# PeterouZh/CIPS-3Dplusplus

Hardware: AMD Instinct MI355X
Metric: rendered views/sec at FFHQ 1024^2 (generator forward: 64x64-ray NeRF + StyleGAN2 decoder) (higher is better)
Workload: dtype f32 (split-fp16 MFMA products x3, f32 accumulate and storage); 1 GPU; ffhq_r1024_nerf64x64x24_D2_B1_fp32; img_size=64, n_samples=24, N_layers_renderer=2, resolution=1024, parallelism=views x1, views_in_flight=2

## Files before the change

### cips_3dplusplus_amd/csrc/fused_stage.hip

```cpp

#include <type_traits>

#include "up2_fir.h"

namespace {

struct FusedArgs {
  const float* y_lo; const float* fir; const float* noise1; int64_t nbs1; const float* nw1; const float* bias1;
  const float* wm2; const float* noise2; int64_t nbs2; const float* nw2; const float* bias2; float* out2;
  const float* wm_rgb; const float* bias_rgb; const float* skip; int skip_up; float* rgb;
  int B, H, W;
  int bf16;
  const float* wm_next; float* y_next;
  const float* x_amax; const float* lconst1; const float* lconst2; float* next_amax;
  float next_gain;
  int flat;
};

#ifndef CIPS3D_FUSED_AB
#define CIPS3D_FUSED_AB 0
#endif
#ifdef CIPS3D_FUSED_STAMPS
__device__ unsigned long long g_fused_stamps[4][8];
#define FSTAMP(i) do { const unsigned long long t_ = __builtin_amdgcn_s_memtime(); fst_[i] += t_ - ftp_; ftp_ = t_; } while (0)
#define FSTAMP_FLUSH() do { if (tid == 0 && (blockIdx.x & 31) == 0) {    constexpr int sl_ = C == 32 ? 0 : C == 64 ? 1 : C == 128 ? 2 : 3; \
    for (int i_ = 0; i_ < 7; ++i_) atomicAdd(&g_fused_stamps[sl_][i_], fst_[i_]); atomicAdd(&g_fused_stamps[sl_][7], 1ull); } } while (0)
#else
#define FSTAMP(i)
#define FSTAMP_FLUSH()
#endif

template <int C, int WM, int WGM, int WGN, int RW, int BK, int MINW, int PREC, bool NEXT = false, bool XPREF = false,
          bool LATE_OPS = false, bool FLAT = false>
__global__ void __launch_bounds__(64 * WGM * WGN, MINW) fused_up_conv_kernel(FusedArgs a) {
  constexpr bool BF16 = PREC == 1 || PREC == 2;
  constexpr bool YB = PREC == 2;
  constexpr bool SPLIT = PREC == 3;
  typedef typename std::conditional<YB, bf16_t, float>::type ylo_t;
  constexpr int NT = 64 * WGM * WGN;
  constexpr int CW = 64 / RW, TH = RW * WGN, TW = CW, BN = TH * TW;
  constexpr int NSTAGE = C / BK, NBUF = NSTAGE > 1 ? 2 : 1, KQ = BK / 16;
  constexpr int LPR = CW / 4;
  static_assert((WGM * WGN == 8 || WGM * WGN == 4) && 16 * WM * WGM == C && TH % 2 == 0 && C % BK == 0, "tile shape");
  constexpr int NBLK = (TH / 2) * (TW / 4);
  constexpr int BPT = BK * NBLK / NT;
  static_assert((BK * NBLK) % NT == 0 && BPT >= 1, "block split");
  __shared__ __attribute__((aligned(16))) float sB[NBUF * BK * BN];
  __shared__ __attribute__((aligned(16))) float s_nz1[BN + 8];
  __shared__ __attribute__((aligned(16))) float s_red_own[NEXT ? WGM * 3 * BN : 4];
  float* s_red = NEXT ? s_red_own : sB;
  __shared__ __attribute__((aligned(16))) float s_wrgb[3 * C];

  const int tid = threadIdx.x;
#ifdef CIPS3D_FUSED_STAMPS
  unsigned long long fst_[7] = {0, 0, 0, 0, 0, 0, 0}, ftp_ = __builtin_amdgcn_s_memtime();
#endif
  const int wave = __builtin_amdgcn_readfirstlane(tid >> 6);
  const int lane = tid & 63;
  const int wm_i = wave / WGN, wn_i = wave % WGN;
  const int q = lane >> 4, jn = lane & 15;
  const int lrow = jn / LPR, lx4 = jn % LPR;
  const int nloc = (wn_i * RW + lrow) * TW + lx4 * 4;
  const int b = blockIdx.z;
  const int H = a.H, W = a.W, OH = FLAT ? H : 2 * H, OW = FLAT ? W : 2 * W;
  const int tiles_x = OW / TW;
  int bid = blockIdx.x;
  if ((gridDim.x & 7) == 0) bid = (bid & 7) * (gridDim.x >> 3) + (bid >> 3);
  const int ox0 = (bid % tiles_x) * TW, oy0 = (bid / tiles_x) * TH;
  const int HWlo = H * W, HWo = OH * OW;
  const int oy = oy0 + wn_i * RW + lrow, ox = ox0 + lx4 * 4;

  float kact1 = 1.41421356237309515f, k2in = kSplitInv, kact2 = 1.41421356237309515f, kback2 = 1.f, kyn = kSplitInv;

  float nw1_u = 0.f;
  float c10_u = 0.f, c11_u = 0.f, c20_u = 0.f, c21a_u = 0.f, c21b_u = 0.f;
  if constexpr (SPLIT) {
    if (a.x_amax && !(CIPS3D_FUSED_AB & 1)) {
      const float* l1 = a.lconst1 + b * 4;
      c10_u = l1[0]; c11_u = l1[1];
      if (NEXT) {
        const float* l2 = a.lconst2 + b * 4;
        c20_u = l2[0]; c21a_u = l2[1]; c21b_u = l2[2];
      }
    }
  }
  const float* ab = a.wm2 + (int64_t)b * C * C;
  f32x4 afr_next[KQ][WM];
#pragma unroll
  for (int kq = 0; kq < KQ; ++kq)
#pragma unroll
    for (int i = 0; i < WM; ++i)
      afr_next[kq][i] = *reinterpret_cast<const f32x4*>(ab + (((wm_i * WM + i) * (C / 16) + kq) * 256 + lane * 4));
  constexpr bool LATE = LATE_OPS;
  f32x4 nz2 = {0.f, 0.f, 0.f, 0.f};
  float nw2_u = 0.f;
  f32x4 bias4[WM];
  auto load_epilogue_ops = [&]() {
    if (a.noise2 && a.nw2 && !(CIPS3D_FUSED_AB & 128)) {
      nz2 = *reinterpret_cast<const f32x4*>(a.noise2 + (int64_t)b * a.nbs2 + (oy * OW + ox));
      nw2_u = a.nw2[0];
    }
#pragma unroll
    for (int i = 0; i < WM; ++i) bias4[i] = *reinterpret_cast<const f32x4*>(a.bias2 + (wm_i * WM + i) * 16 + 4 * q);
  };
  if (!LATE) load_epilogue_ops();

  float kf[16];
#pragma unroll
  for (int i = 0; i < 16; ++i) kf[i] = FLAT ? 0.f : a.fir[15 - i];
  const bool rgb_lane = a.wm_rgb && wm_i == 0 && q < 3;
  float skp[3][4];
  f32x4 skv = {0.f, 0.f, 0.f, 0.f};
  float rgb_bias = 0.f;
  auto load_skip_ops = [&]() {
    if (rgb_lane) {
      rgb_bias = a.bias_rgb[q];
      if (a.skip && !(CIPS3D_FUSED_AB & 128)) {
        if (!FLAT && (a.skip_up & 1)) up2_load(a.skip + (int64_t)b * 3 * HWlo + q * HWlo, H, W, oy >> 1, ox >> 2, skp);
        else skv = *reinterpret_cast<const f32x4*>(a.skip + (int64_t)b * 3 * HWo + (q * HWo + oy * OW + ox));
      }
    }
  };
  if (!LATE) load_skip_ops();

  const bool interior = FLAT || (oy0 / 2 >= 1 && oy0 / 2 + TH / 2 < H && ox0 / 2 >= 1 && ox0 / 2 + TW / 2 < W);
  constexpr bool DEEP = NSTAGE >= 3 && C >= 256;
  float pv[BPT][3][4], pw[BPT][3][4];
  auto patch_load_into = [&](int st, float (&pset)[BPT][3][4]) {
#pragma unroll
    for (int u = 0; u < BPT; ++u) {
      const int g = tid + NT * u;
      const int ch = g / NBLK, rem = g % NBLK;
      const int by = rem / (TW / 4), qx = rem % (TW / 4);
      const ylo_t* src = reinterpret_cast<const ylo_t*>(a.y_lo) + (int64_t)b * C * HWlo + (st * BK + ch) * HWlo;
      if constexpr (CIPS3D_FUSED_AB & 64) {
#pragma unroll
        for (int r = 0; r < 3; ++r)
#pragma unroll
          for (int c = 0; c < 4; ++c) pset[u][r][c] = __int_as_float(0x3c000000 + ((tid + st + r * 4 + c) << 8));
      } else
      if constexpr (FLAT) flat_load(src, W, oy0 + 2 * by, ox0 + 4 * qx, pset[u]);
      else if (interior) up2_load_interior(src, W, oy0 / 2 + by, ox0 / 4 + qx, pset[u]);
      else up2_load(src, H, W, oy0 / 2 + by, ox0 / 4 + qx, pset[u]);
    }
  };
  auto patch_load = [&](int st) { patch_load_into(st, pv); };
  auto patch_store_from = [&](int st, float* dst, float (&pset)[BPT][3][4]) {
#pragma unroll
    for (int u = 0; u < BPT; ++u) {
      const int g = tid + NT * u;
      const int ch = g / NBLK, rem = g % NBLK;
      const int by = rem / (TW / 4), qx = rem % (TW / 4);
      float o[2][4];
      if constexpr (FLAT) {
#pragma unroll
        for (int c = 0; c < 4; ++c) { o[0][c] = pset[u][0][c]; o[1][c] = pset[u][1][c]; }
      } else if constexpr (CIPS3D_FUSED_AB & 8) {
#pragma unroll
        for (int c = 0; c < 4; ++c) { o[0][c] = pset[u][0][c] + pset[u][1][c]; o[1][c] = pset[u][1][c] + pset[u][2][c]; }
      } else {
        up2_fir(pset[u], kf, o);
      }
      const float bs = a.bias1[st * BK + ch];
#pragma unroll
      for (int py = 0; py < 2; ++py) {
        const f32x4 nz = *reinterpret_cast<const f32x4*>(s_nz1 + (2 * by + py) * TW + qx * 4);
        f32x4 v;
#pragma unroll
        for (int c = 0; c < 4; ++c) {
          const float on = fmaf(nw1_u, nz[c], o[py][c]);
          v[c] = (CIPS3D_FUSED_AB & 32) ? on : lrelu02(on + bs);
        }
        if constexpr (SPLIT && !(CIPS3D_FUSED_AB & 32)) {
#pragma unroll
          for (int c = 0; c < 4; ++c) v[c] = pack_split(v[c], kact1);
        } else {
#pragma unroll
          for (int c = 0; c < 4; ++c) v[c] *= kact1;
        }
        *reinterpret_cast<f32x4*>(dst + ch * BN + (2 * by + py) * TW + qx * 4) = v;
      }
    }
  };
  auto patch_store = [&](int st, float* dst) { patch_store_from(st, dst, pv); };
  patch_load(0);
  if (DEEP) patch_load_into(1, pw);
  const bool have_nz = a.noise1 && a.nw1 && !(CIPS3D_FUSED_AB & 128);
  if (have_nz) nw1_u = a.nw1[0];
  if (wave == 0) {
    static_assert(BN / 4 <= 64 && (3 * C) % 4 == 0, "one LDS-DMA instruction per tile");
    if (lane < BN / 4) {
      if (have_nz) {
        const int r = lane / (TW / 4), x4 = lane % (TW / 4);
        __builtin_amdgcn_global_load_lds((const __attribute__((address_space(1))) void*)(a.noise1 + (int64_t)b * a.nbs1 + ((oy0 + r) * OW + ox0 + x4 * 4)),
                                         (__attribute__((address_space(3))) void*)s_nz1, 16, 0, 0);
      } else {
        *reinterpret_cast<f32x4*>(s_nz1 + lane * 4) = f32x4{0.f, 0.f, 0.f, 0.f};
      }
    }
  }
  if (a.wm_rgb) {
#pragma unroll
    for (int p0 = 0; p0 < 3 * C / 4; p0 += 64 * WGM * WGN) {
      const int pbase = p0 + wave * 64;
      if (pbase < 3 * C / 4 && pbase + lane < 3 * C / 4)
        __builtin_amdgcn_global_load_lds((const __attribute__((address_space(1))) void*)(a.wm_rgb + (int64_t)b * 3 * C + (pbase + lane) * 4),
                                         (__attribute__((address_space(3))) void*)(s_wrgb + pbase * 4), 16, 0, 0);
    }
  }


  if constexpr (SPLIT) {
    if (a.x_amax && wave == 0 && !(CIPS3D_FUSED_AB & 1)) {
      const float t = lane < CIPS3D_AMAX_SLOTS ? a.x_amax[b * CIPS3D_AMAX_FLOATS + lane * CIPS3D_AMAX_STRIDE] : 0.f;
      float c10 = c10_u, c11 = c11_u, c20 = 0.f, c21 = 0.f;
      if (NEXT) { c20 = c20_u; c21 = fmaxf(c21a_u, 1.41421356237309515f * c21b_u); }
      if (FLAT) c11 = 1.41421356237309515f;
      const float m_in = cips3d_wave_max_uniform(t);
      const float u1 = fmaf(c11, m_in, c10);
      const int e1 = cips3d_split_exp(u1);
      f32x4 sc = {1.41421356237309515f * cips3d_pow2(-e1), kSplitInv * cips3d_pow2(e1), 1.41421356237309515f, 1.f};
      if (NEXT) {
        const float u2 = fmaf(c21, u1, c20);
        const int e2 = cips3d_split_exp(u2);
        sc[2] = 1.41421356237309515f * cips3d_pow2(-e2);
        sc[3] = cips3d_pow2(e2);
        if (a.next_amax && a.next_gain > 0.f && blockIdx.x == 0 && lane == 0) a.next_amax[b * CIPS3D_AMAX_FLOATS] = a.next_gain * u2 * 1.000001f;
      }
      if (lane == 0) *reinterpret_cast<f32x4*>(s_nz1 + BN) = sc;
    }
  }
  __builtin_amdgcn_s_waitcnt(0x0F70);
  __syncthreads();

  f32x4 acc[WM][4];
#pragma unroll
  for (int i = 0; i < WM; ++i)
#pragma unroll
    for (int c = 0; c < 4; ++c) acc[i][c] = f32x4{0.f, 0.f, 0.f, 0.f};

  FSTAMP(0);
  if constexpr (SPLIT) {
    if (a.x_amax && !(CIPS3D_FUSED_AB & 1)) {
      const f32x4 sc = *reinterpret_cast<const f32x4*>(s_nz1 + BN);
      kact1 = cips3d_uniform(sc[0]);
      k2in = cips3d_uniform(sc[1]);
      if (NEXT) {
        kact2 = cips3d_uniform(sc[2]);
        kback2 = cips3d_uniform(sc[3]);
        kyn = cips3d_uniform(kSplitInv * kback2);
      }
    }
  }

  patch_store(0, sB);
  __syncthreads();
  FSTAMP(1);
#pragma unroll (DEEP ? NSTAGE : 1)
  for (int st = 0; st < NSTAGE; ++st) {
    const float* cur = sB + (NBUF > 1 ? (st & 1) : 0) * BK * BN + nloc;
    f32x4 afr[KQ][WM];
#pragma unroll
    for (int kq = 0; kq < KQ; ++kq)
#pragma unroll
      for (int i = 0; i < WM; ++i) afr[kq][i] = afr_next[kq][i];
    if (st + 1 < NSTAGE) {
#pragma unroll
      for (int kq = 0; kq < KQ; ++kq)
#pragma unroll
        for (int i = 0; i < WM; ++i)
          afr_next[kq][i] = *reinterpret_cast<const f32x4*>(
              ab + (((wm_i * WM + i) * (C / 16) + (st + 1) * KQ + kq) * 256 + lane * 4));
      if (!DEEP) patch_load(st + 1);
    }
    if (DEEP && st + 2 < NSTAGE) {
      if (st & 1) patch_load_into(st + 2, pw);
      else patch_load_into(st + 2, pv);
    }
#pragma unroll
    for (int kq = 0; kq < KQ; ++kq) {
      if (BF16) {
        f32x4 b4[4];
#pragma unroll
        for (int j4 = 0; j4 < 4; ++j4) b4[j4] = *reinterpret_cast<const f32x4*>(cur + (kq * 16 + j4 * 4 + q) * BN);
        s16x4 ah[WM], bh[4];
#pragma unroll
        for (int i = 0; i < WM; ++i) ah[i] = pack_bf16(afr[kq][i][0], afr[kq][i][1], afr[kq][i][2], afr[kq][i][3]);
#pragma unroll
        for (int c = 0; c < 4; ++c) bh[c] = pack_bf16(b4[0][c], b4[1][c], b4[2][c], b4[3][c]);
#pragma unroll
        for (int i = 0; i < WM; ++i)
#pragma unroll
          for (int c = 0; c < 4; ++c)
            acc[i][c] = __builtin_amdgcn_mfma_f32_16x16x16bf16_1k(ah[i], bh[c], acc[i][c], 0, 0, 0);
      } else if constexpr (SPLIT) {
        f32x4 b4[4];
#pragma unroll
        for (int j4 = 0; j4 < 4; ++j4) b4[j4] = *reinterpret_cast<const f32x4*>(cur + (kq * 16 + j4 * 4 + q) * BN);
#pragma unroll
        for (int c = 0; c < 4; ++c) {
          h4 bh, bl;
          unpack_frag(b4[0][c], b4[1][c], b4[2][c], b4[3][c], bh, bl);
#pragma unroll
          for (int i = 0; i < WM; ++i) acc[i][c] = split_mfma16(afr[kq][i], bh, bl, acc[i][c]);
        }
      } else {
#pragma unroll
      for (int j4 = 0; j4 < 4; ++j4) {
        const f32x4 b4 = *reinterpret_cast<const f32x4*>(cur + (kq * 16 + j4 * 4 + q) * BN);
#pragma unroll
        for (int i = 0; i < WM; ++i)
#pragma unroll
          for (int c = 0; c < 4; ++c)
            acc[i][c] = fused_mfma(afr[kq][i][j4], b4[c], acc[i][c]);
      }
      }
    }
    if (NBUF > 1 && st + 1 < NSTAGE) {
      if (DEEP && ((st + 1) & 1)) patch_store_from(st + 1, sB + ((st + 1) & 1) * BK * BN, pw);
      else patch_store(st + 1, sB + ((st + 1) & 1) * BK * BN);
    }
    __syncthreads();
  }

  FSTAMP(2);
  if (LATE) { load_epilogue_ops(); load_skip_ops(); }
  float prgb[3][4];
  float mxn = 0.f;
#pragma unroll
  for (int ch = 0; ch < 3; ++ch)
#pragma unroll
    for (int c = 0; c < 4; ++c) prgb[ch][c] = 0.f;
#pragma unroll
  for (int i = 0; i < WM; ++i) {
    const int obase = (wm_i * WM + i) * 16 + 4 * q;
#pragma unroll
    for (int r = 0; r < 4; ++r) {
      f32x4 v = {acc[i][0][r], acc[i][1][r], acc[i][2][r], acc[i][3][r]};
      if constexpr (SPLIT) {
#pragma unroll
        for (int c = 0; c < 4; ++c) v[c] *= k2in;
      }
#pragma unroll
      for (int c = 0; c < 4; ++c) v[c] = (CIPS3D_FUSED_AB & 16) ? v[c] : lrelu02(fmaf(nw2_u, nz2[c], v[c]) + bias4[i][r]) * kact2;
      if (NEXT) {
#pragma unroll
        for (int c = 0; c < 4; ++c) acc[i][c][r] = v[c];
      }
      if (a.out2) {
        if constexpr (NEXT && SPLIT) {
          *reinterpret_cast<f32x4*>(a.out2 + (int64_t)b * C * HWo + ((obase + r) * HWo + oy * OW + ox)) =
              f32x4{v[0] * kback2, v[1] * kback2, v[2] * kback2, v[3] * kback2};
        } else {
          *reinterpret_cast<f32x4*>(a.out2 + (int64_t)b * C * HWo + ((obase + r) * HWo + oy * OW + ox)) = v;
        }
      }
      if (a.wm_rgb && !(CIPS3D_FUSED_AB & 4)) {
#pragma unroll
        for (int ch = 0; ch < 3; ++ch) {
          const float w = s_wrgb[ch * C + obase + r];
#pragma unroll
          for (int c = 0; c < 4; ++c) prgb[ch][c] = fmaf(w, v[c], prgb[ch][c]);
        }
      }
    }
  }
  FSTAMP(3);
  constexpr int OTN = NEXT ? C / 32 : 1;
  constexpr bool XCHG = NEXT && XPREF && OTN % WGM == 0 && WGM % 2 == 0;
  if (XCHG) {
    constexpr int GR = (WGM / 2) * WM;
    constexpr int TPW = XCHG ? OTN / WGM : 1;
    static_assert(!XCHG || WGN * GR * 4 * 256 <= NBUF * BK * BN, "half of the activations must fit the B stages");
    const float* an = a.wm_next + (int64_t)b * (C / 2) * C + lane * 4;
    float* sx = sB + wn_i * GR * 4 * 256 + lane * 4;
    f32x4 accx[TPW][4];
#pragma unroll
    for (int tp = 0; tp < TPW; ++tp)
#pragma unroll
      for (int c = 0; c < 4; ++c) accx[tp][c] = f32x4{0.f, 0.f, 0.f, 0.f};
#pragma unroll
    for (int rd = 0; rd < 2; ++rd) {
      f32x4 af[TPW][GR];
#pragma unroll
      for (int tp = 0; tp < TPW; ++tp)
#pragma unroll
        for (int gl = 0; gl < GR; ++gl)
          af[tp][gl] = *reinterpret_cast<const f32x4*>(an + ((wm_i * TPW + tp) * (C / 16) + rd * GR + gl) * 256);
      if (wm_i / (WGM / 2) == rd) {
#pragma unroll
        for (int i = 0; i < WM; ++i)
#pragma unroll
          for (int r = 0; r < 4; ++r)
            *reinterpret_cast<f32x4*>(sx + (((wm_i % (WGM / 2)) * WM + i) * 4 + r) * 256) =
                SPLIT ? f32x4{pack_split(acc[i][0][r]), pack_split(acc[i][1][r]), pack_split(acc[i][2][r]), pack_split(acc[i][3][r])}
                      : f32x4{acc[i][0][r], acc[i][1][r], acc[i][2][r], acc[i][3][r]};
      }
      __syncthreads();
#pragma unroll
      for (int gl = 0; gl < GR; ++gl) {
        f32x4 bv[4];
#pragma unroll
        for (int r = 0; r < 4; ++r) bv[r] = *reinterpret_cast<const f32x4*>(sx + (gl * 4 + r) * 256);
        if (BF16) {
          s16x4 bh[4];
#pragma unroll
          for (int c = 0; c < 4; ++c) bh[c] = pack_bf16(bv[0][c], bv[1][c], bv[2][c], bv[3][c]);
#pragma unroll
          for (int tp = 0; tp < TPW; ++tp) {
            const s16x4 ah = pack_bf16(af[tp][gl][0], af[tp][gl][1], af[tp][gl][2], af[tp][gl][3]);
#pragma unroll
            for (int c = 0; c < 4; ++c) accx[tp][c] = __builtin_amdgcn_mfma_f32_16x16x16bf16_1k(ah, bh[c], accx[tp][c], 0, 0, 0);
          }
        } else if constexpr (SPLIT) {
#pragma unroll
          for (int c = 0; c < 4; ++c) {
            h4 bh, bl;
            unpack_frag(bv[0][c], bv[1][c], bv[2][c], bv[3][c], bh, bl);
#pragma unroll
            for (int tp = 0; tp < TPW; ++tp) accx[tp][c] = split_mfma16(af[tp][gl], bh, bl, accx[tp][c]);
          }
        } else {
#pragma unroll
          for (int r = 0; r < 4; ++r)
#pragma unroll
            for (int tp = 0; tp < TPW; ++tp)
#pragma unroll
              for (int c = 0; c < 4; ++c)
                accx[tp][c] = fused_mfma(af[tp][gl][r], bv[r][c], accx[tp][c]);
        }
      }
      __syncthreads();
    }
#pragma unroll
    for (int tp = 0; tp < TPW; ++tp) {
      ylo_t* yn = reinterpret_cast<ylo_t*>(a.y_next) + (int64_t)b * (C / 2) * HWo + (((wm_i * TPW + tp) * 16 + 4 * q) * HWo + oy * OW + ox);
#pragma unroll
      for (int r = 0; r < 4; ++r) {
        const float ys = SPLIT ? kyn : 1.f;
        const f32x4 yv = {accx[tp][0][r] * ys, accx[tp][1][r] * ys, accx[tp][2][r] * ys, accx[tp][3][r] * ys};
        mxn = fmaxf(fmaxf(fmaxf(fabsf(yv[0]), fabsf(yv[1])), fmaxf(fabsf(yv[2]), fabsf(yv[3]))), mxn);
        if constexpr (YB) cips3d_store_wt8(yn + r * HWo, pack_bf16(yv[0], yv[1], yv[2], yv[3]));
        else cips3d_store_wt16(yn + r * HWo, yv);
      }
    }
    if (a.next_amax && !(a.next_gain > 0.f) && !(CIPS3D_FUSED_AB & 2)) {
      static_assert(!NEXT || 4 * WGM * WGN <= BN, "the reduction words fit the noise tile");
      const float m = cips3d_workgroup_max(mxn, s_nz1, wave, lane, WGM * WGN);
      if (tid == 0) cips3d_amax_raise_if(a.next_amax + b * CIPS3D_AMAX_FLOATS, m, blockIdx.x);
    }
  }
  f32x4 accn[OTN][4];
  if (NEXT && !XCHG) {
    static_assert(!NEXT || XCHG || (WGM - 1) * WGN * OTN * 4 * 64 * 4 <= NBUF * BK * BN * 4, "split-K partials must fit the B stages");
    const float* an = a.wm_next + (int64_t)b * (C / 2) * C;
    f32x4 afn[OTN][WM];
#pragma unroll
    for (int t = 0; t < OTN; ++t)
#pragma unroll
      for (int i = 0; i < WM; ++i)
        afn[t][i] = *reinterpret_cast<const f32x4*>(an + ((t * (C / 16) + wm_i * WM + i) * 256 + lane * 4));
#pragma unroll
    for (int t = 0; t < OTN; ++t)
#pragma unroll
      for (int c = 0; c < 4; ++c) accn[t][c] = f32x4{0.f, 0.f, 0.f, 0.f};
#pragma unroll
    for (int i = 0; i < WM; ++i) {
      if (BF16) {
        s16x4 bh[4], ah[OTN];
#pragma unroll
        for (int c = 0; c < 4; ++c) bh[c] = pack_bf16(acc[i][c][0], acc[i][c][1], acc[i][c][2], acc[i][c][3]);
#pragma unroll
        for (int t = 0; t < OTN; ++t) ah[t] = pack_bf16(afn[t][i][0], afn[t][i][1], afn[t][i][2], afn[t][i][3]);
#pragma unroll
        for (int t = 0; t < OTN; ++t)
#pragma unroll
          for (int c = 0; c < 4; ++c) accn[t][c] = __builtin_amdgcn_mfma_f32_16x16x16bf16_1k(ah[t], bh[c], accn[t][c], 0, 0, 0);
      } else if constexpr (SPLIT) {
#pragma unroll
        for (int c = 0; c < 4; ++c) {
          h4 bh, bl;
          split_frag(acc[i][c][0], acc[i][c][1], acc[i][c][2], acc[i][c][3], bh, bl);
#pragma unroll
          for (int t = 0; t < OTN; ++t) accn[t][c] = split_mfma16(afn[t][i], bh, bl, accn[t][c]);
        }
      } else {
#pragma unroll
        for (int r = 0; r < 4; ++r)
#pragma unroll
          for (int t = 0; t < OTN; ++t)
#pragma unroll
            for (int c = 0; c < 4; ++c)
              accn[t][c] = fused_mfma(afn[t][i][r], acc[i][c][r], accn[t][c]);
      }
    }
    if (wm_i > 0) {
      float* sp = sB + ((((wm_i - 1) * WGN + wn_i) * OTN * 4) * 256 + lane * 4);
#pragma unroll
      for (int t = 0; t < OTN; ++t)
#pragma unroll
        for (int c = 0; c < 4; ++c) *reinterpret_cast<f32x4*>(sp + (t * 4 + c) * 256) = accn[t][c];
    }
  }
  FSTAMP(4);
  if (!a.wm_rgb && !NEXT) { FSTAMP_FLUSH(); return; }
  if (a.wm_rgb) {
    if constexpr (MINW >= 8) {
#pragma unroll
      for (int ch = 0; ch < 3; ++ch)
#pragma unroll
        for (int c = 0; c < 4; ++c) {
          float v = prgb[ch][c];
          v += __shfl_xor(v, 16, 64);
          v += __shfl_xor(v, 32, 64);
          prgb[ch][c] = (NEXT && SPLIT) ? v * kback2 : v;
        }
      if (q == 0) {
#pragma unroll
        for (int ch = 0; ch < 3; ++ch)
          *reinterpret_cast<f32x4*>(s_red + (wm_i * 3 + ch) * BN + nloc) =
              f32x4{prgb[ch][0], prgb[ch][1], prgb[ch][2], prgb[ch][3]};
      }
    } else {
    f32x4 tot;
#pragma unroll
    for (int c = 0; c < 4; ++c) {
      const auto rg = __builtin_amdgcn_permlane16_swap(__float_as_uint(prgb[0][c]), __float_as_uint(prgb[1][c]), false, false);
      const auto bb = __builtin_amdgcn_permlane16_swap(__float_as_uint(prgb[2][c]), __float_as_uint(prgb[2][c]), false, false);
      const float p = __uint_as_float(rg[0]) + __uint_as_float(rg[1]);
      const float u = __uint_as_float(bb[0]) + __uint_as_float(bb[1]);
      const auto h = __builtin_amdgcn_permlane32_swap(__float_as_uint(p), __float_as_uint(u), false, false);
      const float v = __uint_as_float(h[0]) + __uint_as_float(h[1]);
      tot[c] = (NEXT && SPLIT) ? v * kback2 : v;
    }
    if (q < 3) *reinterpret_cast<f32x4*>(s_red + (wm_i * 3 + q) * BN + nloc) = tot;
    }
  }
  __syncthreads();
  if (NEXT && !XCHG && wm_i == 0) {
#pragma unroll
    for (int m = 1; m < WGM; ++m) {
      const float* sp = sB + ((((m - 1) * WGN + wn_i) * OTN * 4) * 256 + lane * 4);
#pragma unroll
      for (int t = 0; t < OTN; ++t)
#pragma unroll
        for (int c = 0; c < 4; ++c) {
          const f32x4 pv4 = *reinterpret_cast<const f32x4*>(sp + (t * 4 + c) * 256);
#pragma unroll
          for (int r = 0; r < 4; ++r) accn[t][c][r] += pv4[r];
        }
    }
    ylo_t* yn = reinterpret_cast<ylo_t*>(a.y_next) + (int64_t)b * (C / 2) * HWo + (oy * OW + ox);
#pragma unroll
    for (int t = 0; t < OTN; ++t)
#pragma unroll
      for (int r = 0; r < 4; ++r) {
        const float ys = SPLIT ? kyn : 1.f;
        const f32x4 yv = {accn[t][0][r] * ys, accn[t][1][r] * ys, accn[t][2][r] * ys, accn[t][3][r] * ys};
        mxn = fmaxf(fmaxf(fmaxf(fabsf(yv[0]), fabsf(yv[1])), fmaxf(fabsf(yv[2]), fabsf(yv[3]))), mxn);
        if constexpr (YB) cips3d_store_wt8(yn + (t * 16 + 4 * q + r) * HWo, pack_bf16(yv[0], yv[1], yv[2], yv[3]));
        else cips3d_store_wt16(yn + (t * 16 + 4 * q + r) * HWo, yv);
      }
  }
  if (NEXT && !XCHG && a.next_amax && !(a.next_gain > 0.f) && !(CIPS3D_FUSED_AB & 2)) {
    const float m = cips3d_workgroup_max(mxn, s_nz1, wave, lane, WGM * WGN);
    if (tid == 0) cips3d_amax_raise_if(a.next_amax + b * CIPS3D_AMAX_FLOATS, m, blockIdx.x);
  }
  FSTAMP(5);
  if (!a.wm_rgb) { FSTAMP_FLUSH(); return; }
  if (rgb_lane) {
    const int ch = q;
    f32x4 v = {0.f, 0.f, 0.f, 0.f};
#pragma unroll
    for (int m = 0; m < WGM; ++m) {
      const f32x4 t = *reinterpret_cast<const f32x4*>(s_red + (m * 3 + ch) * BN + nloc);
#pragma unroll
      for (int c = 0; c < 4; ++c) v[c] += t[c];
    }
#pragma unroll
    for (int c = 0; c < 4; ++c) v[c] += rgb_bias;
    if (a.skip) {
      if (!FLAT && (a.skip_up & 1)) {
        float so[2][4];
        up2_fir(skp, kf, so);
        const int py = oy & 1;
#pragma unroll
        for (int c = 0; c < 4; ++c) v[c] += py ? so[1][c] : so[0][c];
      } else {
#pragma unroll
        for (int c = 0; c < 4; ++c) v[c] += skv[c];
      }
    }
    if (a.skip_up & 2) {
      unsigned pk = 0;
#pragma unroll
      for (int c = 0; c < 4; ++c) {
        const float cl = fminf(fmaxf(v[c], -1.f), 1.f);
        pk |= (unsigned)__float2int_rn((cl + 1.f) * 127.5f) << (8 * c);
      }
      *reinterpret_cast<unsigned*>(reinterpret_cast<unsigned char*>(a.rgb) + (int64_t)b * 3 * HWo + (ch * HWo + oy * OW + ox)) = pk;
    } else {
      cips3d_store_wt16(a.rgb + (int64_t)b * 3 * HWo + (ch * HWo + oy * OW + ox), v);
    }
  }
  FSTAMP(6);
  FSTAMP_FLUSH();
}

template <int C, int WM, int WGM, int WGN, int RW, int BK, int MINW, bool NEXT, bool XPREF, bool LATE, bool FLAT>
int launch_fused_as(const FusedArgs& a, hipStream_t st) {
  constexpr int TH = RW * WGN, TW = 64 / RW;
  const int up = FLAT ? 1 : 2;
  dim3 grid((unsigned)((up * a.W / TW) * (up * a.H / TH)), 1, (unsigned)a.B);
  if (a.bf16 == 3) hipLaunchKernelGGL((fused_up_conv_kernel<C, WM, WGM, WGN, RW, BK, MINW, 3, NEXT, XPREF, LATE, FLAT>), grid, dim3(64 * WGM * WGN), 0, st, a);
  else if (a.bf16 == 2) hipLaunchKernelGGL((fused_up_conv_kernel<C, WM, WGM, WGN, RW, BK, MINW, 2, NEXT, XPREF, LATE, FLAT>), grid, dim3(64 * WGM * WGN), 0, st, a);
  else if (a.bf16) hipLaunchKernelGGL((fused_up_conv_kernel<C, WM, WGM, WGN, RW, BK, MINW, 1, NEXT, XPREF, LATE, FLAT>), grid, dim3(64 * WGM * WGN), 0, st, a);
  else hipLaunchKernelGGL((fused_up_conv_kernel<C, WM, WGM, WGN, RW, BK, MINW, 0, NEXT, XPREF, LATE, FLAT>), grid, dim3(64 * WGM * WGN), 0, st, a);
  return cips3d_launch_status();
}
template <int C, int WM, int WGM, int WGN, int RW, int BK, int MINW, bool NEXT = false, bool XPREF = false, bool LATE = false>
int launch_fused(const FusedArgs& a, hipStream_t st) {
  return a.flat ? launch_fused_as<C, WM, WGM, WGN, RW, BK, MINW, NEXT, XPREF, LATE, true>(a, st)
                : launch_fused_as<C, WM, WGM, WGN, RW, BK, MINW, NEXT, XPREF, LATE, false>(a, st);
}

}

#ifdef CIPS3D_FUSED_STAMPS
extern "C" int cips3d_debug_read_fused_stamps(unsigned long long* out32) {
  hipDeviceSynchronize();
  hipMemcpyFromSymbol(out32, HIP_SYMBOL(g_fused_stamps), 256);
  unsigned long long z[32] = {0};
  hipMemcpyToSymbol(HIP_SYMBOL(g_fused_stamps), z, 256);
  return 0;
}
#endif

extern "C" int cips3d_fused_up_conv_supported(int C, int H, int W) {
  return (C == 32 || C == 64 || C == 128 || C == 256) && W % 32 == 0 && H % 2 == 0 && H >= 2 &&
         (int64_t)C * 4 * H * W < ((int64_t)1 << 31);
}

extern "C" int cips3d_fused_flat_conv_supported(int C, int H, int W) {
  return (C == 32 || C == 64 || C == 128 || C == 256) && W % 64 == 0 && H % 4 == 0 && H >= 4 &&
         (int64_t)C * H * W < ((int64_t)1 << 31);
}

extern "C" int cips3d_fused_up_conv(const float* y_lo, const float* fir, const float* noise1, int64_t noise1_bstride,
                                    const float* noise_w1, const float* bias1, const float* wm2, const float* noise2,
                                    int64_t noise2_bstride, const float* noise_w2, const float* bias2, float* out2,
                                    const float* wm_rgb, const float* bias_rgb, const float* skip, int skip_up,
                                    float* rgb, int B, int C, int H, int W, const cips3d_range* rg, void* stream) {
  return cips3d_fused_up_conv_next(y_lo, fir, noise1, noise1_bstride, noise_w1, bias1, wm2, noise2, noise2_bstride, noise_w2,
                                   bias2, out2, wm_rgb, bias_rgb, skip, skip_up, rgb, nullptr, nullptr, B, C, H, W, rg, stream);
}

extern "C" int cips3d_fused_up_conv_chains(int C) { return C == 64 || C == 128 || C == 256; }

extern "C" int cips3d_fused_up_conv_next(const float* y_lo, const float* fir, const float* noise1, int64_t noise1_bstride,
                                         const float* noise_w1, const float* bias1, const float* wm2, const float* noise2,
                                         int64_t noise2_bstride, const float* noise_w2, const float* bias2, float* out2,
                                         const float* wm_rgb, const float* bias_rgb, const float* skip, int skip_up,
                                         float* rgb, const float* wm_next, float* y_next, int B, int C, int H, int W,
                                         const cips3d_range* rg, void* stream) {
  const int flat = (skip_up & CIPS3D_STAGE_FLAT) ? 1 : 0;
  if (!y_lo || (!fir && !flat) || !bias1 || !wm2 || !bias2 || B < 0 || H <= 0 || W <= 0) return CIPS3D_E_BADARG;
  if (flat && (skip_up & 1)) return CIPS3D_E_BADARG;
  if ((wm_next == nullptr) != (y_next == nullptr)) return CIPS3D_E_BADARG;
  if (wm_next && !cips3d_fused_up_conv_chains(C)) return CIPS3D_E_UNSUPP;
  if (!out2 && !wm_rgb && !wm_next) return CIPS3D_E_BADARG;
  if (wm_rgb && (!bias_rgb || !rgb)) return CIPS3D_E_BADARG;
  if (!(flat ? cips3d_fused_flat_conv_supported(C, H, W) : cips3d_fused_up_conv_supported(C, H, W))) return CIPS3D_E_UNSUPP;
  if (B == 0) return 0;
  FusedArgs a{y_lo, fir, noise1, noise1_bstride, noise_w1, bias1, wm2, noise2, noise2_bstride, noise_w2, bias2, out2,
              wm_rgb, bias_rgb, skip, (skip_up & 1) | ((skip_up & CIPS3D_RGB_U8) ? 2 : 0), rgb, B, H, W,
              (skip_up & CIPS3D_GEMM_SPLIT) ? 3 : (skip_up & CIPS3D_GEMM_BF16) ? ((skip_up & CIPS3D_Y_BF16) ? 2 : 1) : 0, wm_next,
              y_next, rg ? rg->x_amax : nullptr, rg ? rg->lconst : nullptr, rg ? rg->lconst2 : nullptr,
              rg ? rg->next_amax : nullptr, rg ? rg->next_gain : 0.f, flat};
  if ((skip_up & CIPS3D_GEMM_SPLIT) && rg && rg->x_amax && (!rg->lconst || (wm_next && !rg->lconst2))) return CIPS3D_E_BADARG;
  if ((skip_up & CIPS3D_Y_BF16) && !(skip_up & CIPS3D_GEMM_BF16)) return CIPS3D_E_BADARG;
  if ((skip_up & CIPS3D_GEMM_SPLIT) && (skip_up & CIPS3D_GEMM_BF16)) return CIPS3D_E_BADARG;
  hipStream_t st = as_stream(stream);
  if (wm_next)
    return C == 64    ? launch_fused<64, 2, 2, 2, 1, 16, 4, true, true, true>(a, st)
           : C == 128 ? launch_fused<128, 4, 2, 2, 1, 32, 2, true, false, true>(a, st)
                      : launch_fused<256, 2, 8, 1, 2, 64, 2, true, true>(a, st);
  switch (C) {
    case 32: return launch_fused<32, 1, 2, 2, 1, 32, 8, false, false, true>(a, st);
    case 64: return launch_fused<64, 2, 2, 2, 1, 16, 4>(a, st);
    case 128: return launch_fused<128, 4, 2, 4, 1, 32, 2>(a, st);
    case 256: return launch_fused<256, 2, 8, 1, 2, 64, 2>(a, st);
  }
  return CIPS3D_E_UNSUPP;
}
```

### cips_3dplusplus_amd/csrc/up2_fir.h

```cpp
#pragma once
#include "mfma_frag.h"

__device__ __forceinline__ float up2_tap(const float* __restrict__ src, int H, int W, int oy, int ox,
                                         const float* __restrict__ fir) {
  const int ky0 = oy & 1, kx0 = ox & 1;
  float acc = 0.f;
#pragma unroll
  for (int a = 0; a < 2; ++a) {
    const int ky = ky0 + 2 * a;
    const int iy = (oy + ky - 2) >> 1;
    if (iy < 0 || iy >= H) continue;
#pragma unroll
    for (int c = 0; c < 2; ++c) {
      const int kx = kx0 + 2 * c;
      const int ix = (ox + kx - 2) >> 1;
      if (ix < 0 || ix >= W) continue;
      acc = fmaf(src[(int64_t)iy * W + ix], fir[15 - (ky * 4 + kx)], acc);
    }
  }
  return acc;
}

__device__ __forceinline__ void up2_load_interior(const float* __restrict__ src, int W, int iy, int qx, float (&v)[3][4]) {
  const float* row = src + ((iy - 1) * W + 2 * qx);
#pragma unroll
  for (int r = 0; r < 3; ++r) {
    const float2 mid = *reinterpret_cast<const float2*>(row);
    v[r][0] = row[-1]; v[r][1] = mid.x; v[r][2] = mid.y; v[r][3] = row[2];
    row += W;
  }
}

typedef unsigned short bf16_t;
__device__ __forceinline__ float bf16_f32(unsigned bits) { return __uint_as_float(bits << 16); }
__device__ __forceinline__ void up2_load_interior(const bf16_t* __restrict__ src, int W, int iy, int qx, float (&v)[3][4]) {
  const bf16_t* row = src + ((iy - 1) * W + 2 * qx);
#pragma unroll
  for (int r = 0; r < 3; ++r) {
    const unsigned mid = *reinterpret_cast<const unsigned*>(row);
    v[r][0] = bf16_f32(row[-1]); v[r][1] = bf16_f32(mid & 0xffffu); v[r][2] = __uint_as_float(mid & 0xffff0000u);
    v[r][3] = bf16_f32(row[2]);
    row += W;
  }
}
__device__ __forceinline__ void up2_load(const bf16_t* __restrict__ src, int H, int W, int iy, int qx, float (&v)[3][4]) {
  const int c = 2 * qx;
#pragma unroll
  for (int r = 0; r < 3; ++r) {
    const int y = iy - 1 + r;
    const bool yok = (y >= 0) && (y < H);
    const bf16_t* row = src + (yok ? y : 0) * W;
    unsigned mid = 0u;
    if (yok) mid = *reinterpret_cast<const unsigned*>(row + c);
    v[r][1] = bf16_f32(mid & 0xffffu); v[r][2] = __uint_as_float(mid & 0xffff0000u);
    v[r][0] = (yok && c - 1 >= 0) ? bf16_f32(row[c - 1]) : 0.f;
    v[r][3] = (yok && c + 2 < W) ? bf16_f32(row[c + 2]) : 0.f;
  }
}

__device__ __forceinline__ void up2_load(const float* __restrict__ src, int H, int W, int iy, int qx, float (&v)[3][4]) {
  const int c = 2 * qx;
#pragma unroll
  for (int r = 0; r < 3; ++r) {
    const int y = iy - 1 + r;
    const bool yok = (y >= 0) && (y < H);
    const float* row = src + (yok ? y : 0) * W;
    float2 mid = make_float2(0.f, 0.f);
    if (yok) mid = *reinterpret_cast<const float2*>(row + c);
    v[r][1] = mid.x; v[r][2] = mid.y;
    v[r][0] = (yok && c - 1 >= 0) ? row[c - 1] : 0.f;
    v[r][3] = (yok && c + 2 < W) ? row[c + 2] : 0.f;
  }
}

__device__ __forceinline__ void flat_load(const float* __restrict__ src, int W, int y, int x, float (&v)[3][4]) {
#pragma unroll
  for (int r = 0; r < 2; ++r) {
    const f32x4 t = *reinterpret_cast<const f32x4*>(src + ((y + r) * W + x));
#pragma unroll
    for (int c = 0; c < 4; ++c) v[r][c] = t[c];
  }
}
__device__ __forceinline__ void flat_load(const bf16_t* __restrict__ src, int W, int y, int x, float (&v)[3][4]) {
#pragma unroll
  for (int r = 0; r < 2; ++r) {
    const uint2 t = *reinterpret_cast<const uint2*>(src + ((y + r) * W + x));
    v[r][0] = bf16_f32(t.x & 0xffffu); v[r][1] = __uint_as_float(t.x & 0xffff0000u);
    v[r][2] = bf16_f32(t.y & 0xffffu); v[r][3] = __uint_as_float(t.y & 0xffff0000u);
  }
}

__device__ __forceinline__ void up2_fir(const float (&v)[3][4], const float (&kf)[16], float (&o)[2][4]) {
#pragma unroll
  for (int py = 0; py < 2; ++py) {
#pragma unroll
    for (int j = 0; j < 4; ++j) {
      const int px = j & 1;
      const int col0 = (j + 1) >> 1;
      float acc = 0.f;
#pragma unroll
      for (int a = 0; a < 2; ++a) {
        const int ky = py + 2 * a;
        const int r = py + a;
#pragma unroll
        for (int bb = 0; bb < 2; ++bb) acc = fmaf(v[r][col0 + bb], kf[ky * 4 + px + 2 * bb], acc);
      }
      o[py][j] = acc;
    }
  }
}
```

Before: 3385 views/s.

## Use 32-bit offset addressing, trimmed skip loads, and swizzle reductions in fused stage

Global loads and stores switch to scalar-base plus unsigned 32-bit offsets via up2_at and an inline-asm global_store_dwordx4 with sc1, aiming to cut 64-bit address arithmetic and VGPR use. The skip upsample path for RW==1 now loads only the two input rows each output row needs, uses a single unaligned 16-byte load on interior tiles, and computes one FIR row instead of two. The skip-operand load moves after the epilogue when NEXT is set, which shortens register live ranges. The cross-lane RGB reduction replaces shfl_xor with ds_swizzle and ds_bpermute. Risks are 32-bit offset overflow on large tensors and correctness of the hand-written asm store and swizzle pattern.

After: 3397 views/s, median of 2. Within noise of the previous version (+0.3%).

```diff
diff --git a/cips_3dplusplus_amd/csrc/fused_stage.hip b/cips_3dplusplus_amd/csrc/fused_stage.hip
--- a/cips_3dplusplus_amd/csrc/fused_stage.hip
+++ b/cips_3dplusplus_amd/csrc/fused_stage.hip
@@ -29,6 +29,12 @@
 #define FSTAMP(i)
 #define FSTAMP_FLUSH()
 #endif
+
+template <class T16>
+__device__ __forceinline__ void store_wt16_at(void* ubase, unsigned boff, T16 v) {
+  static_assert(sizeof(T16) == 16, "16-byte payload");
+  asm volatile("global_store_dwordx4 %0, %1, %2 sc1\n\ts_nop 1" :: "v"(boff), "v"(__builtin_bit_cast(f32x4, v)), "s"(ubase) : "memory");
+}
 
 template <int C, int WM, int WGM, int WGN, int RW, int BK, int MINW, int PREC, bool NEXT = false, bool XPREF = false,
           bool LATE_OPS = false, bool FLAT = false>
@@ -90,14 +96,14 @@
   for (int kq = 0; kq < KQ; ++kq)
 #pragma unroll
     for (int i = 0; i < WM; ++i)
-      afr_next[kq][i] = *reinterpret_cast<const f32x4*>(ab + (((wm_i * WM + i) * (C / 16) + kq) * 256 + lane * 4));
+      afr_next[kq][i] = *reinterpret_cast<const f32x4*>(up2_at(ab, (unsigned)(((wm_i * WM + i) * (C / 16) + kq) * 256 + lane * 4)));
   constexpr bool LATE = LATE_OPS;
   f32x4 nz2 = {0.f, 0.f, 0.f, 0.f};
   float nw2_u = 0.f;
   f32x4 bias4[WM];
   auto load_epilogue_ops = [&]() {
     if (a.noise2 && a.nw2 && !(CIPS3D_FUSED_AB & 128)) {
-      nz2 = *reinterpret_cast<const f32x4*>(a.noise2 + (int64_t)b * a.nbs2 + (oy * OW + ox));
+      nz2 = *reinterpret_cast<const f32x4*>(up2_at(a.noise2 + (int64_t)b * a.nbs2, (unsigned)(oy * OW + ox)));
       nw2_u = a.nw2[0];
     }
 #pragma unroll
@@ -108,7 +114,9 @@
   float kf[16];
 #pragma unroll
   for (int i = 0; i < 16; ++i) kf[i] = FLAT ? 0.f : a.fir[15 - i];
+  const bool interior = FLAT || (oy0 / 2 >= 1 && oy0 / 2 + TH / 2 < H && ox0 / 2 >= 1 && ox0 / 2 + TW / 2 < W);
   const bool rgb_lane = a.wm_rgb && wm_i == 0 && q < 3;
+  constexpr bool SKIP2 = !FLAT && RW == 1;
   float skp[3][4];
   f32x4 skv = {0.f, 0.f, 0.f, 0.f};
   float rgb_bias = 0.f;
@@ -116,14 +124,16 @@
     if (rgb_lane) {
       rgb_bias = a.bias_rgb[q];
       if (a.skip && !(CIPS3D_FUSED_AB & 128)) {
-        if (!FLAT && (a.skip_up & 1)) up2_load(a.skip + (int64_t)b * 3 * HWlo + q * HWlo, H, W, oy >> 1, ox >> 2, skp);
-        else skv = *reinterpret_cast<const f32x4*>(a.skip + (int64_t)b * 3 * HWo + (q * HWo + oy * OW + ox));
+        const int siy = (oy >> 1) + (SKIP2 ? (oy & 1) : 0);
+        if (!FLAT && (a.skip_up & 1) && interior)
+          up2_load_interior_at<SKIP2 ? 2 : 3>(a.skip + (int64_t)b * 3 * HWlo, (unsigned)(q * HWlo + (siy - 1) * W + 2 * (ox >> 2)), W, skp);
+        else if (!FLAT && (a.skip_up & 1)) up2_load_at<SKIP2 ? 2 : 3>(a.skip + (int64_t)b * 3 * HWlo, (unsigned)(q * HWlo), H, W, siy, ox >> 2, skp);
+        else skv = *reinterpret_cast<const f32x4*>(up2_at(a.skip + (int64_t)b * 3 * HWo, (unsigned)(q * HWo + oy * OW + ox)));
       }
     }
   };
   if (!LATE) load_skip_ops();
 
-  const bool interior = FLAT || (oy0 / 2 >= 1 && oy0 / 2 + TH / 2 < H && ox0 / 2 >= 1 && ox0 / 2 + TW / 2 < W);
   constexpr bool DEEP = NSTAGE >= 3 && C >= 256;
   float pv[BPT][3][4], pw[BPT][3][4];
   auto patch_load_into = [&](int st, float (&pset)[BPT][3][4]) {
@@ -270,7 +280,7 @@
 #pragma unroll
         for (int i = 0; i < WM; ++i)
           afr_next[kq][i] = *reinterpret_cast<const f32x4*>(
-              ab + (((wm_i * WM + i) * (C / 16) + (st + 1) * KQ + kq) * 256 + lane * 4));
+              up2_at(ab, (unsigned)(((wm_i * WM + i) * (C / 16) + (st + 1) * KQ + kq) * 256 + lane * 4)));
       if (!DEEP) patch_load(st + 1);
     }
     if (DEEP && st + 2 < NSTAGE) {
@@ -324,7 +334,7 @@
   }
 
   FSTAMP(2);
-  if (LATE) { load_epilogue_ops(); load_skip_ops(); }
+  if (LATE) { load_epilogue_ops(); if (!NEXT) load_skip_ops(); }
   float prgb[3][4];
   float mxn = 0.f;
 #pragma unroll
@@ -348,12 +358,9 @@
         for (int c = 0; c < 4; ++c) acc[i][c][r] = v[c];
       }
       if (a.out2) {
-        if constexpr (NEXT && SPLIT) {
-          *reinterpret_cast<f32x4*>(a.out2 + (int64_t)b * C * HWo + ((obase + r) * HWo + oy * OW + ox)) =
-              f32x4{v[0] * kback2, v[1] * kback2, v[2] * kback2, v[3] * kback2};
-        } else {
-          *reinterpret_cast<f32x4*>(a.out2 + (int64_t)b * C * HWo + ((obase + r) * HWo + oy * OW + ox)) = v;
-        }
+        f32x4* o2 = reinterpret_cast<f32x4*>(a.out2 + (int64_t)b * C * HWo + ((obase + r) * HWo + oy * OW + ox));
+        if constexpr (NEXT && SPLIT) *o2 = f32x4{v[0] * kback2, v[1] * kback2, v[2] * kback2, v[3] * kback2};
+        else *o2 = v;
       }
       if (a.wm_rgb && !(CIPS3D_FUSED_AB & 4)) {
 #pragma unroll
@@ -365,6 +372,7 @@
       }
     }
   }
+  if (LATE && NEXT) load_skip_ops();
   FSTAMP(3);
   constexpr int OTN = NEXT ? C / 32 : 1;
   constexpr bool XCHG = NEXT && XPREF && OTN % WGM == 0 && WGM % 2 == 0;
@@ -434,14 +442,15 @@
     }
 #pragma unroll
     for (int tp = 0; tp < TPW; ++tp) {
-      ylo_t* yn = reinterpret_cast<ylo_t*>(a.y_next) + (int64_t)b * (C / 2) * HWo + (((wm_i * TPW + tp) * 16 + 4 * q) * HWo + oy * OW + ox);
+      ylo_t* yn_b = reinterpret_cast<ylo_t*>(a.y_next) + (int64_t)b * (C / 2) * HWo;
+      const unsigned yo = (unsigned)(((wm_i * TPW + tp) * 16 + 4 * q) * HWo + oy * OW + ox);
 #pragma unroll
       for (int r = 0; r < 4; ++r) {
         const float ys = SPLIT ? kyn : 1.f;
         const f32x4 yv = {accx[tp][0][r] * ys, accx[tp][1][r] * ys, accx[tp][2][r] * ys, accx[tp][3][r] * ys};
         mxn = fmaxf(fmaxf(fmaxf(fabsf(yv[0]), fabsf(yv[1])), fmaxf(fabsf(yv[2]), fabsf(yv[3]))), mxn);
-        if constexpr (YB) cips3d_store_wt8(yn + r * HWo, pack_bf16(yv[0], yv[1], yv[2], yv[3]));
-        else cips3d_store_wt16(yn + r * HWo, yv);
+        if constexpr (YB) cips3d_store_wt8(up2_at(yn_b, yo + (unsigned)(r * HWo)), pack_bf16(yv[0], yv[1], yv[2], yv[3]));
+        else store_wt16_at(yn_b, (yo + (unsigned)(r * HWo)) * (unsigned)sizeof(ylo_t), yv);
       }
     }
     if (a.next_amax && !(a.next_gain > 0.f) && !(CIPS3D_FUSED_AB & 2)) {
@@ -511,8 +520,8 @@
 #pragma unroll
         for (int c = 0; c < 4; ++c) {
           float v = prgb[ch][c];
-          v += __shfl_xor(v, 16, 64);
-          v += __shfl_xor(v, 32, 64);
+          v += __int_as_float(__builtin_amdgcn_ds_swizzle(__float_as_int(v), 0x401F));
+          v += __int_as_float(__builtin_amdgcn_ds_bpermute((lane << 2) ^ 128, __float_as_int(v)));
           prgb[ch][c] = (NEXT && SPLIT) ? v * kback2 : v;
         }
       if (q == 0) {
@@ -550,7 +559,8 @@
           for (int r = 0; r < 4; ++r) accn[t][c][r] += pv4[r];
         }
     }
-    ylo_t* yn = reinterpret_cast<ylo_t*>(a.y_next) + (int64_t)b * (C / 2) * HWo + (oy * OW + ox);
+    ylo_t* yn_b = reinterpret_cast<ylo_t*>(a.y_next) + (int64_t)b * (C / 2) * HWo;
+    const unsigned yo = (unsigned)(4 * q * HWo + oy * OW + ox);
 #pragma unroll
     for (int t = 0; t < OTN; ++t)
 #pragma unroll
@@ -558,8 +568,8 @@
         const float ys = SPLIT ? kyn : 1.f;
         const f32x4 yv = {accn[t][0][r] * ys, accn[t][1][r] * ys, accn[t][2][r] * ys, accn[t][3][r] * ys};
         mxn = fmaxf(fmaxf(fmaxf(fabsf(yv[0]), fabsf(yv[1])), fmaxf(fabsf(yv[2]), fabsf(yv[3]))), mxn);
-        if constexpr (YB) cips3d_store_wt8(yn + (t * 16 + 4 * q + r) * HWo, pack_bf16(yv[0], yv[1], yv[2], yv[3]));
-        else cips3d_store_wt16(yn + (t * 16 + 4 * q + r) * HWo, yv);
+        if constexpr (YB) cips3d_store_wt8(up2_at(yn_b, yo + (unsigned)((t * 16 + r) * HWo)), pack_bf16(yv[0], yv[1], yv[2], yv[3]));
+        else store_wt16_at(yn_b, (yo + (unsigned)((t * 16 + r) * HWo)) * (unsigned)sizeof(ylo_t), yv);
       }
   }
   if (NEXT && !XCHG && a.next_amax && !(a.next_gain > 0.f) && !(CIPS3D_FUSED_AB & 2)) {
@@ -580,7 +590,13 @@
 #pragma unroll
     for (int c = 0; c < 4; ++c) v[c] += rgb_bias;
     if (a.skip) {
-      if (!FLAT && (a.skip_up & 1)) {
+      if (SKIP2 && (a.skip_up & 1)) {
+        float so[4];
+        if (oy & 1) up2_fir_row<1>(skp, kf, so);
+        else up2_fir_row<0>(skp, kf, so);
+#pragma unroll
+        for (int c = 0; c < 4; ++c) v[c] += so[c];
+      } else if (!FLAT && (a.skip_up & 1)) {
         float so[2][4];
         up2_fir(skp, kf, so);
         const int py = oy & 1;
@@ -600,7 +616,7 @@
       }
       *reinterpret_cast<unsigned*>(reinterpret_cast<unsigned char*>(a.rgb) + (int64_t)b * 3 * HWo + (ch * HWo + oy * OW + ox)) = pk;
     } else {
-      cips3d_store_wt16(a.rgb + (int64_t)b * 3 * HWo + (ch * HWo + oy * OW + ox), v);
+      store_wt16_at(a.rgb + (int64_t)b * 3 * HWo, (unsigned)(ch * HWo + oy * OW + ox) * 4u, v);
     }
   }
   FSTAMP(6);
diff --git a/cips_3dplusplus_amd/csrc/up2_fir.h b/cips_3dplusplus_amd/csrc/up2_fir.h
--- a/cips_3dplusplus_amd/csrc/up2_fir.h
+++ b/cips_3dplusplus_amd/csrc/up2_fir.h
@@ -28,6 +28,21 @@
     const float2 mid = *reinterpret_cast<const float2*>(row);
     v[r][0] = row[-1]; v[r][1] = mid.x; v[r][2] = mid.y; v[r][3] = row[2];
     row += W;
+  }
+}
+
+template <class T>
+__device__ __forceinline__ T* up2_at(T* ubase, unsigned off) {
+  return (T*)((const char*)ubase + off * (unsigned)sizeof(T));
+}
+template <int NR = 3>
+__device__ __forceinline__ void up2_load_interior_at(const float* __restrict__ ubase, unsigned off, int W, float (&v)[3][4]) {
+  typedef float f32x4_a4 __attribute__((ext_vector_type(4), aligned(4)));
+#pragma unroll
+  for (int r = 0; r < NR; ++r) {
+    const f32x4_a4 t = *reinterpret_cast<const f32x4_a4*>(up2_at(ubase, off) - 1);
+    v[r][0] = t[0]; v[r][1] = t[1]; v[r][2] = t[2]; v[r][3] = t[3];
+    off += (unsigned)W;
   }
 }
 
@@ -73,6 +88,22 @@
   }
 }
 
+template <int NR = 3>
+__device__ __forceinline__ void up2_load_at(const float* __restrict__ ubase, unsigned poff, int H, int W, int iy, int qx, float (&v)[3][4]) {
+  const int c = 2 * qx;
+#pragma unroll
+  for (int r = 0; r < NR; ++r) {
+    const int y = iy - 1 + r;
+    const bool yok = (y >= 0) && (y < H);
+    const float* row = up2_at(ubase, poff + (unsigned)((yok ? y : 0) * W + c));
+    float2 mid = make_float2(0.f, 0.f);
+    if (yok) mid = *reinterpret_cast<const float2*>(row);
+    v[r][1] = mid.x; v[r][2] = mid.y;
+    v[r][0] = (yok && c - 1 >= 0) ? row[-1] : 0.f;
+    v[r][3] = (yok && c + 2 < W) ? row[2] : 0.f;
+  }
+}
+
 __device__ __forceinline__ void flat_load(const float* __restrict__ src, int W, int y, int x, float (&v)[3][4]) {
 #pragma unroll
   for (int r = 0; r < 2; ++r) {
@@ -87,6 +118,24 @@
     const uint2 t = *reinterpret_cast<const uint2*>(src + ((y + r) * W + x));
     v[r][0] = bf16_f32(t.x & 0xffffu); v[r][1] = __uint_as_float(t.x & 0xffff0000u);
     v[r][2] = bf16_f32(t.y & 0xffffu); v[r][3] = __uint_as_float(t.y & 0xffff0000u);
+  }
+}
+
+template <int PY>
+__device__ __forceinline__ void up2_fir_row(const float (&v)[3][4], const float (&kf)[16], float (&o)[4]) {
+#pragma unroll
+  for (int j = 0; j < 4; ++j) {
+    const int px = j & 1;
+    const int col0 = (j + 1) >> 1;
+    float acc = 0.f;
+#pragma unroll
+    for (int a = 0; a < 2; ++a) {
+#pragma unroll
+      for (int bb = 0; bb < 2; ++bb) {
+        acc = fmaf(v[a][col0 + bb], kf[(PY + 2 * a) * 4 + px + 2 * bb], acc);
+      }
+    }
+    o[j] = acc;
   }
 }
 
```
